# TFMV/quiver

Measured on AMD Instinct MI355X. Metric: flat_cosine_qps_recall_1.0, higher is better.
Workload: dtype f64; 1 GPU; flat cosine scan 10000000x768 fp32, k=10, single query per step, recall 1.0 (exact, bit-identical to the CPU oracle); rows_total=10000000, rows_per_gpu=10000000, dim=768, k=10, scan_streams=1, device=AMD Radeon Graphics (gfx950:sramecc+:xnack-), cus=256, rccl_ranks_seen=0

## Files before the change

### quiver_amd/csrc/qv_bound_scan.hip

```cpp
#include "qv_kernels.h"
#include "qv_bound.h"

namespace qv {

typedef uint32_t u4 __attribute__((ext_vector_type(4)));
constexpr uint32_t kBoundCandCap = 4096;
constexpr uint32_t kBoundMaxDim = 4096;
struct BoundCtrl { uint32_t thr_inv, cand_cnt, ticket, flag; };

template <int U, bool QN>
__device__ __forceinline__ void bound_block(const u4* __restrict__ p, const float* __restrict__ q_lds, uint32_t s0, float& acc, double& qa) {
    u4 x[2 * U];
#pragma unroll
    for (int u = 0; u < U; u++) {
        x[2 * u] = __builtin_nontemporal_load(&p[(size_t)(s0 + u) * 128]);
        x[2 * u + 1] = __builtin_nontemporal_load(&p[(size_t)(s0 + u) * 128 + 32]);
    }
    __builtin_amdgcn_sched_barrier(0);
#pragma unroll
    for (int u = 0; u < U; u++) {
        const f4* qq = reinterpret_cast<const f4*>(q_lds + (size_t)(s0 + u) * 16);
#pragma unroll
        for (int h = 0; h < 2; h++) {
            const u4 w = x[2 * u + h];
            const f4 qa4 = qq[2 * h], qb4 = qq[2 * h + 1];
            const float qe[8] = {qa4.x, qa4.y, qa4.z, qa4.w, qb4.x, qb4.y, qb4.z, qb4.w};
            const uint32_t ww[4] = {w.x, w.y, w.z, w.w};
#pragma unroll
            for (int j = 0; j < 4; j++) {
                acc = __builtin_fmaf(qe[2 * j], __uint_as_float(ww[j] << 16), acc);
                acc = __builtin_fmaf(qe[2 * j + 1], __uint_as_float(ww[j] & 0xFFFF0000u), acc);
                if constexpr (QN) { const double a = (double)qe[2 * j], b = (double)qe[2 * j + 1]; qa = __builtin_fma(a, a, qa); qa = __builtin_fma(b, b, qa); }
            }
        }
    }
}
template <bool QN>
__device__ __forceinline__ float bound_tile(const u4* __restrict__ p, const float* __restrict__ q_lds, uint32_t steps, double* qn2) {
    float acc = 0.f; double qa = 0.0;
    uint32_t s = 0;
    for (; s + 8 <= steps; s += 8) bound_block<8, QN>(p, q_lds, s, acc, qa);
    if (s + 4 <= steps) { bound_block<4, QN>(p, q_lds, s, acc, qa); s += 4; }
    if (s + 2 <= steps) { bound_block<2, QN>(p, q_lds, s, acc, qa); s += 2; }
    if (s < steps) bound_block<1, QN>(p, q_lds, s, acc, qa);
    if constexpr (QN) *qn2 = qa;
    return acc;
}

__device__ __forceinline__ bool bound_scan_tail(uint64_t list, uint64_t thr, uint64_t* wl , uint32_t wave, uint32_t lane, uint32_t k, BoundCtrl* __restrict__ ctrl,
                                                uint64_t* __restrict__ partial, uint32_t* __restrict__ seed_rows, float* __restrict__ seed_dist) {
    __shared__ uint32_t s_last;
    const uint32_t kth = k - 1;
    wl[wave * 64 + lane] = list;
    __syncthreads();
    if (wave == 0) {
        for (uint32_t w = 1; w < kScanWaves; w++) list_insert(list, thr, lane < k ? wl[w * 64 + lane] : kDeadKey, kth, lane);
        uint64_t* mine = partial + (size_t)blockIdx.x * k;
        if (lane < k) (void)atomicExch(reinterpret_cast<unsigned long long*>(&mine[lane]), (unsigned long long)list);
        asm volatile("s_waitcnt vmcnt(0)" ::: "memory");
        uint32_t last = 0;
        if (lane == 0) last = atomicAdd(&ctrl->ticket, 1u) == gridDim.x - 1 ? 1u : 0u;
        last = __builtin_amdgcn_readfirstlane(last);
        if (last && lane == 0) ctrl->ticket = 0;
        if (lane == 0) s_last = last;
    }
    __syncthreads();
    if (!s_last) return false;
    merge_lists_last_workgroup(partial, gridDim.x, k, seed_rows, seed_dist);
    if (wave == 0 && lane == kth) {
        const uint32_t o = ord_f32(seed_dist[kth]);
        ctrl->thr_inv = (seed_rows[kth] != 0xFFFFFFFFu && o < 0xFF800000u) ? ~o : 0u;
        ctrl->cand_cnt = 0;
    }
    return true;
}

template <int M, bool SKIP = false>
__global__ void __launch_bounds__(kScanBlock)
k_bound_scan(IndexView v, const float* __restrict__ query, uint32_t k, BoundCtrl* __restrict__ ctrl, uint32_t* __restrict__ lo_all ,
             uint64_t* __restrict__ partial , uint32_t* __restrict__ seed_rows, float* __restrict__ seed_dist,
             const uint32_t* __restrict__ gate = nullptr ) {
    if (gate != nullptr && *gate == 0u) return;
    extern __shared__ __align__(16) unsigned char smem[];
    float* q_lds = reinterpret_cast<float*>(smem);
    uint64_t* wl = reinterpret_cast<uint64_t*>(smem + (size_t)v.dim * sizeof(float));
    const uint32_t lane = lane_id();
    const uint32_t wave = __builtin_amdgcn_readfirstlane(threadIdx.x >> 6);
    for (uint32_t i = threadIdx.x; i < v.dim; i += blockDim.x) q_lds[i] = query[i];
    __syncthreads();
    const uint32_t steps = v.dim >> 4, tw = gridDim.x * kScanWaves, kth = k - 1;
    const double gamma = bound_scan_gamma(v.dim);
    const u4* plane = reinterpret_cast<const u4*>(v.plane) + ((lane >> 5) * 64 + (lane & 31));
    uint64_t list = kDeadKey, thr = kDeadKey;
    double qn = 0.0;

    uint64_t am_read = 0ull;
    auto finish_tile = [&](uint32_t t, float s, bool first) {
        const uint32_t row = t * 64 + lane;
        const double rn = v.rnorm[row];
        const float rr = v.rres[row];
        uint64_t am;
        if constexpr (SKIP) am = am_read; else am = v.alive[t];
        float lo, hi;
        (void)bound_scan_interval<M>(s, qn, rn, rr, v.dim, gamma, lo, hi);
        const bool live = (am >> lane) & 1ull;
        __builtin_nontemporal_store(live ? ord_f32(lo) : 0xFFFFFFFFu, &lo_all[row]);
        const uint64_t key = live ? (((uint64_t)ord_f32(hi) << 32) | row) : kDeadKey;
        if (first) { list = wave_sort64(key, lane); thr = readlane64(list, kth); }
        else list_insert(list, thr, key, kth, lane);
    };

    uint32_t t = blockIdx.x * kScanWaves + wave;
    if constexpr (SKIP) {
        bool first = true;
        uint64_t am_next = t < v.n_tiles ? v.alive[t] : 0ull;
        for (; t < v.n_tiles; t += tw) {
            const uint64_t am = am_next;
            if (t + tw < v.n_tiles) am_next = v.alive[t + tw];
            if (am == 0ull) { __builtin_nontemporal_store(0xFFFFFFFFu, &lo_all[t * 64 + lane]); continue; }
            am_read = am;
            if (first) {
                double qn2 = 0.0;
                const float s = bound_tile<true>(plane + (size_t)t * steps * 128, q_lds, steps, &qn2);
                qn = __builtin_sqrt(qn2);
                finish_tile(t, s, true);
                first = false;
            } else finish_tile(t, bound_tile<false>(plane + (size_t)t * steps * 128, q_lds, steps, nullptr), false);
        }
    } else {
        if (t < v.n_tiles) {
            double qn2 = 0.0;
            const float s = bound_tile<true>(plane + (size_t)t * steps * 128, q_lds, steps, &qn2);
            qn = __builtin_sqrt(qn2);
            finish_tile(t, s, true);
            t += tw;
        }
        for (; t < v.n_tiles; t += tw) finish_tile(t, bound_tile<false>(plane + (size_t)t * steps * 128, q_lds, steps, nullptr), false);
    }

    (void)bound_scan_tail(list, thr, wl, wave, lane, k, ctrl, partial, seed_rows, seed_dist);
}

__device__ __forceinline__ void bound_collect(const uint32_t* __restrict__ lo, uint32_t n , uint32_t H, uint32_t* __restrict__ cnt, uint32_t* __restrict__ cand,
                                              uint32_t cap = kBoundCandCap, const uint32_t* __restrict__ ids = nullptr) {
    const uint32_t lane = lane_id();
    for (uint32_t base = blockIdx.x * 1024u; base < n; base += gridDim.x * 1024u) {
        const uint32_t i = base + threadIdx.x * 4u;
        u4 x = {0xFFFFFFFFu, 0xFFFFFFFFu, 0xFFFFFFFFu, 0xFFFFFFFFu};
        if (i < n) x = __builtin_nontemporal_load(reinterpret_cast<const u4*>(lo + i));
        const uint32_t xs[4] = {x.x, x.y, x.z, x.w};
#pragma unroll
        for (int j = 0; j < 4; j++) {
            const bool c = xs[j] <= H && xs[j] != 0xFFFFFFFFu;
            const uint64_t m = __ballot(c);
            if (m) {
                uint32_t b0 = 0;
                if (lane == (uint32_t)__builtin_ctzll(m)) b0 = atomicAdd(cnt, (uint32_t)__builtin_popcountll(m));
                b0 = __builtin_amdgcn_readlane(b0, (uint32_t)__builtin_ctzll(m));
                const uint32_t slot = b0 + (uint32_t)__builtin_popcountll(m & ((1ull << lane) - 1ull));
                if (c && slot < cap) cand[slot] = ids ? ids[i + (uint32_t)j] : i + (uint32_t)j;
            }
        }
    }
}
__global__ void __launch_bounds__(256)
k_bound_collect(const uint32_t* __restrict__ lo_all, uint32_t n , BoundCtrl* __restrict__ ctrl, uint32_t* __restrict__ cand,
                const uint32_t* __restrict__ gate = nullptr , uint32_t cap = kBoundCandCap,
                const uint32_t* __restrict__ n_ptr = nullptr ,
                const uint32_t* __restrict__ ids = nullptr ) {
    if (gate != nullptr && *gate == 0u) return;
    const uint32_t inv = ctrl->thr_inv;
    if (inv == 0u) return;
    if (n_ptr != nullptr) n = *n_ptr;
    bound_collect(lo_all, n, ~inv, &ctrl->cand_cnt, cand, cap, ids);
}

template <int M, typename F>
__device__ __forceinline__ void bound_rescore_query(const IndexView& v, const float* __restrict__ query, uint32_t k, uint32_t cnt, bool has_H, const uint32_t* __restrict__ cand,
                                                    uint32_t* __restrict__ rows_out, float* __restrict__ dist_out, F decided) {
    using Q = typename MT<M>::Q;
    extern __shared__ __align__(16) unsigned char smem[];
    Q* q_lds = reinterpret_cast<Q*>(smem);
    uint64_t* wl = reinterpret_cast<uint64_t*>(smem + (((size_t)v.dim4 * 4 * sizeof(Q)) + 15) / 16 * 16);
    __shared__ double s_qn;
    const uint32_t lane = lane_id();
    const uint32_t wave = __builtin_amdgcn_readfirstlane(threadIdx.x >> 6);
    const uint32_t ns = cnt < kBoundCandCap ? cnt : kBoundCandCap, kth = k - 1;
    stage_query<M>(q_lds, query, v.dim, v.dim4);
    __syncthreads();
    const f4* tiles = reinterpret_cast<const f4*>(v.tiles);
    if (wave == kScanWaves - 1) {
        double ma = 0.0;
        for (uint32_t i = 0; i < v.dim; i++) { const double a = (double)q_lds[i]; ma = __builtin_fma(a, a, ma); }
        if (lane == 0) s_qn = __builtin_sqrt(ma);
    }
    __syncthreads();
    const double qn = s_qn;
    const bool hand_back = cnt > kBoundCandCap || !has_H || !bound_scan_norm_ok(qn, v.dim);
    if (threadIdx.x == 0) decided(hand_back);
    if (hand_back) return;
    QConst qc; qc.qn = 0.0; qc.qn32 = 0.0f;
    if constexpr (M == QV_COSINE) qc.qn = qn;
    uint64_t list = kDeadKey, thr = kDeadKey;
    for (uint32_t base = wave * 64; base < ns; base += kScanWaves * 64) {
        const uint32_t i = base + lane;
        uint64_t key = kDeadKey;
        if (i < ns) {
            const uint32_t row = cand[i];
            const typename MT<M>::A acc = row_accumulate<M, kUnroll, false, true>(tiles + (size_t)(row >> 6) * v.dim4 * 64 + (row & 63), 64, q_lds, v.dim4);
            double rn = 0.0;
            if constexpr (MT<M>::needs_rnorm) rn = v.rnorm[row];
            key = make_key(finalize<M>(acc, qc, rn), row);
        }
        if (base == wave * 64) { list = wave_sort64(key, lane); thr = readlane64(list, kth); }
        else list_insert(list, thr, key, kth, lane);
    }
    __syncthreads();
    wl[wave * 64 + lane] = list;
    __syncthreads();
    if (wave == 0) {
        for (uint32_t w = 1; w < kScanWaves; w++) list_insert(list, thr, lane < k ? wl[w * 64 + lane] : kDeadKey, kth, lane);
        if (lane < k) {
            const bool dead = list == kDeadKey;
            rows_out[lane] = dead ? 0xFFFFFFFFu : (uint32_t)list;
            dist_out[lane] = dead ? __uint_as_float(0x7F800000u) : unord_f32((uint32_t)(list >> 32));
        }
    }
}

constexpr uint32_t kBoundRescoreGrid = 64;
constexpr uint32_t kBoundRefineGrid = 256;
template <int M, bool P8 = false>
__global__ void __launch_bounds__(kScanBlock)
k_bound_rescore(IndexView v, const float* __restrict__ query, uint32_t k, BoundCtrl* __restrict__ ctrl, const uint32_t* __restrict__ cand,
                uint32_t* __restrict__ stats, uint32_t* __restrict__ rows_out, float* __restrict__ dist_out, uint32_t* gate, BoundCtrl* next,
                uint64_t* __restrict__ partial ) {
    if (gate != nullptr && *gate == 0u) return;
    using Q = typename MT<M>::Q;
    extern __shared__ __align__(16) unsigned char smem[];
    Q* q_lds = reinterpret_cast<Q*>(smem);
    const size_t q_bytes = (((size_t)v.dim4 * 4 * sizeof(Q)) + 15) / 16 * 16;
    uint64_t* wl = reinterpret_cast<uint64_t*>(smem + q_bytes);
    float* rbuf = reinterpret_cast<float*>(smem + q_bytes + (size_t)kScanWaves * 64 * sizeof(uint64_t));
    __shared__ double s_qn;
    __shared__ uint32_t s_last;
    const uint32_t cnt = ctrl->cand_cnt, thr_inv = ctrl->thr_inv;
    const uint32_t lane = lane_id();
    const uint32_t wave = __builtin_amdgcn_readfirstlane(threadIdx.x >> 6);
    const uint32_t ns = cnt < kBoundCandCap ? cnt : kBoundCandCap, kth = k - 1;
    const uint32_t active = std::max(1u, std::min((uint32_t)gridDim.x, (ns + kScanWaves - 1) / kScanWaves));
    const bool idle = blockIdx.x >= active;
    if (idle) {
        if (threadIdx.x == 0) s_last = atomicAdd(&ctrl->ticket, 1u) == gridDim.x - 1 ? 1u : 0u;
        __syncthreads();
        if (!s_last) return;
    }
    stage_query<M>(q_lds, query, v.dim, v.dim4);
    __syncthreads();
    if (wave == kScanWaves - 1) {
        double ma = 0.0;
        for (uint32_t i = 0; i < v.dim; i++) { const double a = (double)q_lds[i]; ma = __builtin_fma(a, a, ma); }
        if (lane == 0) s_qn = __builtin_sqrt(ma);
    }
    __syncthreads();
    const double qn = s_qn;
    const bool hand_back = cnt > kBoundCandCap || thr_inv == 0u || !bound_scan_norm_ok(qn, v.dim);
    uint64_t list = kDeadKey, thr = kDeadKey;
    if (!hand_back && !idle) {
        QConst qc; qc.qn = 0.0; qc.qn32 = 0.0f;
        if constexpr (M == QV_COSINE) qc.qn = qn;
        const f4* tiles = reinterpret_cast<const f4*>(v.tiles);
        f4* mine = reinterpret_cast<f4*>(rbuf + (size_t)wave * v.dim4 * 4);
        bool first = true;
        for (uint32_t i = blockIdx.x * kScanWaves + wave; i < ns; i += active * kScanWaves) {
            const uint32_t row = cand[i];
            const f4* src = tiles + (size_t)(row >> 6) * v.dim4 * 64 + (row & 63);
            double rn = 0.0;
            if constexpr (MT<M>::needs_rnorm) rn = v.rnorm[row];
            for (uint32_t c0 = 0; c0 < v.dim4; c0 += 256) {
                f4 x[4];
#pragma unroll
                for (uint32_t u = 0; u < 4; u++) { const uint32_t c = c0 + u * 64 + lane; if (c < v.dim4) x[u] = __builtin_nontemporal_load(&src[(size_t)c * 64]); }
#pragma unroll
                for (uint32_t u = 0; u < 4; u++) { const uint32_t c = c0 + u * 64 + lane; if (c < v.dim4) mine[c] = x[u]; }
            }
            __builtin_amdgcn_fence(__ATOMIC_RELEASE, "wavefront");
            __builtin_amdgcn_wave_barrier();
            __builtin_amdgcn_fence(__ATOMIC_ACQUIRE, "wavefront");
            typename MT<M>::A acc = 0;
            for (uint32_t c = 0; c < v.dim4; c++) {
                const f4 r = mine[c];
                const Q* qq = q_lds + (size_t)c * 4;
                acc1<M>(acc, qq[0], r.x); acc1<M>(acc, qq[1], r.y); acc1<M>(acc, qq[2], r.z); acc1<M>(acc, qq[3], r.w);
            }
            __builtin_amdgcn_fence(__ATOMIC_RELEASE, "wavefront");
            __builtin_amdgcn_wave_barrier();
            const uint64_t key = lane == 0 ? make_key(finalize<M>(acc, qc, rn), row) : kDeadKey;
            if (first) { list = wave_sort64(key, lane); thr = readlane64(list, kth); first = false; }
            else list_insert(list, thr, key, kth, lane);
        }
    }
    wl[wave * 64 + lane] = list;
    __syncthreads();
    if (wave == 0 && !idle) {
        if (!hand_back) {
            for (uint32_t w = 1; w < kScanWaves; w++) list_insert(list, thr, lane < k ? wl[w * 64 + lane] : kDeadKey, kth, lane);
            uint64_t* out = partial + (size_t)blockIdx.x * k;
            if (lane < k) (void)atomicExch(reinterpret_cast<unsigned long long*>(&out[lane]), (unsigned long long)list);
            asm volatile("s_waitcnt vmcnt(0)" ::: "memory");
        }
        uint32_t last = 0;
        if (lane == 0) last = atomicAdd(&ctrl->ticket, 1u) == gridDim.x - 1 ? 1u : 0u;
        last = __builtin_amdgcn_readfirstlane(last);
        if (lane == 0) s_last = last;
    }
    __syncthreads();
    if (!s_last) return;
    if (threadIdx.x == 0) {
        ctrl->ticket = 0;
        if constexpr (P8) {
            stats[kBound8StatsWord] = cnt;
            if (hand_back) (void)atomicAdd(&stats[kBound8StatsWord + 1], 1u);
            (void)atomicAdd(&stats[kBound8StatsWord + 2], 1u);
            if (!hand_back) { stats[0] = cnt; (void)atomicAdd(&stats[2], 1u); next->flag = 0u; }
        } else {
            stats[0] = cnt;
            if (hand_back) (void)atomicAdd(&stats[1], 1u);
            (void)atomicAdd(&stats[2], 1u);
            if (gate != nullptr) *gate = 0u;
        }
        ctrl->flag = hand_back ? 1u : 0u;
        ctrl->cand_cnt = 0; ctrl->thr_inv = 0;
    }
    if (hand_back) return;
    merge_lists_last_workgroup(partial, active, k, rows_out, dist_out);
}

typedef int i32;
template <int U>
__device__ __forceinline__ void bound8_block(const u4* __restrict__ p, const u4* __restrict__ qh, const u4* __restrict__ ql, uint32_t s0, i32 (&acc)[4]) {
    u4 x[U];
#pragma unroll
// ... 45 lines not shown
    double r2 = 0.0;
    int qs = 0;
    for (uint32_t i = threadIdx.x; i < dim; i += blockDim.x) {
        const double x = q_ok ? (double)query[i] : 0.0;
        const double qq = __builtin_rint(x / sq);
        const double hi = __builtin_rint(qq * (1.0 / 128.0)), lo = qq - 128.0 * hi;
        qh8[i] = (int8_t)(int)hi; ql8[i] = (int8_t)(int)lo;
        if constexpr (SUM) qs += (int)qq;
        const double d = x - sq * qq;
        r2 = __builtin_fma(d, d, r2);
    }
    r2 = wave_sum_f64(r2);
    if (lane == 0) s_res[wave] = r2;
    if constexpr (SUM) {
#pragma unroll
        for (int m = 32; m >= 1; m >>= 1) qs += __shfl_xor(qs, m);
        if (lane == 0) s_sum[wave] = qs;
    }
    if (wave == kScanWaves - 1) {
        double ma = 0.0;
        for (uint32_t b = 0; b < dim; b += 64) {
            const float x = b + lane < dim ? query[b + lane] : 0.f;
            const uint32_t n = dim - b < 64u ? dim - b : 64u;
            for (uint32_t j = 0; j < n; j++) { const double a = (double)__uint_as_float(__builtin_amdgcn_readlane(__float_as_uint(x), j)); ma = __builtin_fma(a, a, ma); }
        }
        if (lane == 0) s_qn = __builtin_sqrt(ma);
    }
    __syncthreads();
    double qres2 = 0.0;
    for (uint32_t w = 0; w < kScanWaves; w++) qres2 += s_res[w];
    qn_out = s_qn;
    sq_out = sq;
    qres_out = q_ok ? __builtin_sqrt(qres2) * (1.0 + 1e-9) + 1e-300 : __builtin_nan("");
    qsum_out = 0;
    if constexpr (SUM) { for (uint32_t w = 0; w < kScanWaves; w++) qsum_out += (long long)s_sum[w]; }
}

template <int M, bool SKIP = false>
__global__ void __launch_bounds__(kScanBlock)
k_bound_scan8(IndexView v, const float* __restrict__ query, uint32_t k, BoundCtrl* __restrict__ ctrl, uint32_t* __restrict__ lo_all ,
              uint64_t* __restrict__ partial , uint32_t* __restrict__ seed_rows, float* __restrict__ seed_dist) {
    extern __shared__ __align__(16) unsigned char smem[];
    int8_t* qh8 = reinterpret_cast<int8_t*>(smem);
    int8_t* ql8 = qh8 + v.dim;
    uint64_t* wl = reinterpret_cast<uint64_t*>(smem + (size_t)v.dim * 2);
    const uint32_t lane = lane_id();
    const uint32_t wave = __builtin_amdgcn_readfirstlane(threadIdx.x >> 6);
    const uint32_t steps = v.dim >> 4, tw = gridDim.x * kScanWaves;
    double sq, qn, qres; long long qsum;
    bound8_stage_query<false>(query, v.dim, qh8, ql8, lane, wave, sq, qn, qres, qsum);

    const u4* qh = reinterpret_cast<const u4*>(qh8);
    const u4* ql = reinterpret_cast<const u4*>(ql8);
    const u4* plane = reinterpret_cast<const u4*>(v.plane8) + lane;
    const uint32_t kth = k - 1;
    uint64_t list = kDeadKey, thr = kDeadKey;
    bool first = true;
    uint32_t t = blockIdx.x * kScanWaves + wave;
    uint64_t am_next = 0ull;
    if constexpr (SKIP) am_next = t < v.n_tiles ? v.alive[t] : 0ull;
    for (; t < v.n_tiles; t += tw) {
        uint64_t am;
        if constexpr (SKIP) {
            am = am_next;
            if (t + tw < v.n_tiles) am_next = v.alive[t + tw];
            if (am == 0ull) { __builtin_nontemporal_store(0xFFFFFFFFu, &lo_all[t * 64 + lane]); continue; }
        }
        const uint32_t row = t * 64 + lane;
        const double rn = v.rnorm[row];
        const float sc = v.rscale8[row], rr = v.rres8[row];
        if constexpr (!SKIP) am = v.alive[t];
        const long long isum = bound8_tile(plane + (size_t)t * steps * 64, qh, ql, steps);
        float lo, hi;
        (void)bound_scan_interval8<M>(isum, sq, qn, qres, rn, sc, rr, v.dim, lo, hi);
        const bool live = (am >> lane) & 1ull;
        __builtin_nontemporal_store(live ? ord_f32(lo) : 0xFFFFFFFFu, &lo_all[row]);
        const uint64_t key = live ? (((uint64_t)ord_f32(hi) << 32) | row) : kDeadKey;
        if (first) { list = wave_sort64(key, lane); thr = readlane64(list, kth); first = false; }
        else list_insert(list, thr, key, kth, lane);
    }
    (void)bound_scan_tail(list, thr, wl, wave, lane, k, ctrl, partial, seed_rows, seed_dist);
}

struct BoundQuery8 { double sq, qn, qres, pad; int8_t terms[2 * kBoundMaxDim]; };
template <int U>
__device__ __forceinline__ void bound6_block(const u4* __restrict__ p, const u4* __restrict__ qh, const u4* __restrict__ ql, uint32_t g0, i32 (&acc)[4]) {
    u4 x[3 * U];
#pragma unroll
    for (int u = 0; u < 3 * U; u++) x[u] = __builtin_nontemporal_load(&p[((size_t)g0 * 3 + u) * 64]);
    __builtin_amdgcn_sched_barrier(0);
#pragma unroll
    for (int u = 0; u < U; u++) {
        const uint32_t X[4] = {x[3 * u].x, x[3 * u].y, x[3 * u].z, x[3 * u].w};
        const uint32_t Y[4] = {x[3 * u + 1].x, x[3 * u + 1].y, x[3 * u + 1].z, x[3 * u + 1].w};
        const uint32_t Z[4] = {x[3 * u + 2].x, x[3 * u + 2].y, x[3 * u + 2].z, x[3 * u + 2].w};
        uint32_t c[4][4];
#pragma unroll
        for (int j = 0; j < 4; j++) {
            c[0][j] = X[j] & 0x3F3F3F3Fu; c[1][j] = Y[j] & 0x3F3F3F3Fu; c[2][j] = Z[j] & 0x3F3F3F3Fu;
            c[3][j] = ((X[j] >> 6) & 0x03030303u) | ((Y[j] >> 4) & 0x0C0C0C0Cu) | ((Z[j] >> 2) & 0x30303030u);
        }
#pragma unroll
        for (int st = 0; st < 4; st++) {
            const u4 h = qh[(g0 + u) * 4 + st], l = ql[(g0 + u) * 4 + st];
            acc[0] = __builtin_amdgcn_sdot4((i32)h.x, (i32)c[st][0], acc[0], false);
            acc[1] = __builtin_amdgcn_sdot4((i32)h.y, (i32)c[st][1], acc[1], false);
            acc[0] = __builtin_amdgcn_sdot4((i32)h.z, (i32)c[st][2], acc[0], false);
            acc[1] = __builtin_amdgcn_sdot4((i32)h.w, (i32)c[st][3], acc[1], false);
            acc[2] = __builtin_amdgcn_sdot4((i32)l.x, (i32)c[st][0], acc[2], false);
            acc[3] = __builtin_amdgcn_sdot4((i32)l.y, (i32)c[st][1], acc[3], false);
            acc[2] = __builtin_amdgcn_sdot4((i32)l.z, (i32)c[st][2], acc[2], false);
            acc[3] = __builtin_amdgcn_sdot4((i32)l.w, (i32)c[st][3], acc[3], false);
        }
    }
}
__device__ __forceinline__ long long bound6_tile(const u4* __restrict__ p, const u4* __restrict__ qh, const u4* __restrict__ ql, uint32_t groups) {
    i32 acc[4] = {0, 0, 0, 0};
    uint32_t g = 0;
    for (; g + 6 <= groups; g += 6) bound6_block<6>(p, qh, ql, g, acc);
    if (g + 3 <= groups) { bound6_block<3>(p, qh, ql, g, acc); g += 3; }
    if (g + 2 <= groups) { bound6_block<2>(p, qh, ql, g, acc); g += 2; }
    if (g < groups) bound6_block<1>(p, qh, ql, g, acc);
    return ((long long)acc[0] + (long long)acc[1]) * 128ll + ((long long)acc[2] + (long long)acc[3]);
}

template <int M>
__global__ void __launch_bounds__(kScanBlock)
k_bound_scan6(IndexView v, const float* __restrict__ query, uint32_t k, BoundCtrl* __restrict__ ctrl, uint32_t* __restrict__ lo_all ,
              uint64_t* __restrict__ partial , uint32_t* __restrict__ seed_rows, float* __restrict__ seed_dist,
              BoundQuery8* __restrict__ qst ) {
    extern __shared__ __align__(16) unsigned char smem[];
    int8_t* qh8 = reinterpret_cast<int8_t*>(smem);
    int8_t* ql8 = qh8 + v.dim;
    uint64_t* wl = reinterpret_cast<uint64_t*>(smem + (size_t)v.dim * 2);
    const uint32_t lane = lane_id();
    const uint32_t wave = __builtin_amdgcn_readfirstlane(threadIdx.x >> 6);
    const uint32_t groups = v.dim >> 6, tw = gridDim.x * kScanWaves;
    double sq, qn, qres; long long qsum;
    bound8_stage_query<true>(query, v.dim, qh8, ql8, lane, wave, sq, qn, qres, qsum);
    const long long bias = (long long)kBound6Bias * qsum;
    if (blockIdx.x == 0) {
        for (uint32_t i = threadIdx.x; i < v.dim / 8; i += blockDim.x) reinterpret_cast<u4*>(qst->terms)[i] = reinterpret_cast<const u4*>(smem)[i];
        if (threadIdx.x == 0) { qst->sq = sq; qst->qn = qn; qst->qres = qres; }
    }

    const u4* qh = reinterpret_cast<const u4*>(qh8);
    const u4* ql = reinterpret_cast<const u4*>(ql8);
    const u4* plane = reinterpret_cast<const u4*>(v.plane6) + lane;
    const uint32_t kth = k - 1;
    uint64_t list = kDeadKey, thr = kDeadKey;
    bool first = true;
    for (uint32_t t = blockIdx.x * kScanWaves + wave; t < v.n_tiles; t += tw) {
        const uint32_t row = t * 64 + lane;
        const double rn = v.rnorm[row];
        const float sc = 4.0f * v.rscale8[row], rr = v.rres6[row];
        const uint64_t am = v.alive[t];
        const long long isum = bound6_tile(plane + (size_t)t * groups * 192, qh, ql, groups) - bias;
        float lo, hi;
        (void)bound_scan_interval8<M>(isum, sq, qn, qres, rn, sc, rr, v.dim, lo, hi);
        const bool live = (am >> lane) & 1ull;
        __builtin_nontemporal_store(live ? ord_f32(lo) : 0xFFFFFFFFu, &lo_all[row]);
        const uint64_t key = live ? (((uint64_t)ord_f32(hi) << 32) | row) : kDeadKey;
        if (first) { list = wave_sort64(key, lane); thr = readlane64(list, kth); first = false; }
        else list_insert(list, thr, key, kth, lane);
    }
    (void)bound_scan_tail(list, thr, wl, wave, lane, k, ctrl, partial, seed_rows, seed_dist);
}
// ... 487 lines not shown
    for (int c = 0; c < 3; c++) {
        const BoundFloor &b = kBoundFloor[kRulesBf16][c], &l = kBoundFloor[kRulesBf16L2][c], &p = kBoundFloor[kRulesPlane8][c];
        const BoundFilterFloor& pf = kBoundFilterFloor[kRulesPlane8][c];
        if (p.wide_rows < b.wide_rows || p.wide_rows < l.wide_rows || p.narrow_dim < b.narrow_dim || p.narrow_dim < l.narrow_dim) return false;
        if (p.narrow_rows != 0 && (p.narrow_rows < b.narrow_rows || p.narrow_rows < l.narrow_rows)) return false;
        if (pf.min_dim < kBound8MinDim || (pf.min_rows != 0 && pf.min_rows < p.wide_rows)) return false;
    }
    return true;
}
static_assert(bound_floors_nest(), "the 8-bit floors are never below the bound scan's own, class by class, and its filtered floors never below its unfiltered ones");
static int rule_metric(const IndexView& v) { return v.metric == QV_L2 && v.l2_planes ? QV_RULE_L2_PLANES : v.metric; }
BoundAsk bound_ask(const IndexView& v, uint32_t nq, uint32_t k, uint32_t candidate_tiles) {
    return {rule_metric(v), v.dim, v.n_rows, nq, k, candidate_tiles, v.plane != nullptr, v.plane8 != nullptr, v.plane8 != nullptr && v.plane6 != nullptr};
}
BoundKnobs bound_knobs(const IndexView& v) { return {v.bound_scan, {v.bound_plane, v.bound_plane_filtered, v.bound_plane_mq, v.bound_plane_filtered_mq}, v.bound_plane6}; }
int bound_scan_mode(int mode) { static const int env_mode = env_int("QV_BOUND_SCAN", 0); return mode ? mode : env_mode; }
static int bound_plane_mode(BoundForm form, int mode) {
    static const int env_mode[4] = {env_int("QV_BOUND_PLANE", 0), env_int("QV_BOUND_PLANE_FILTERED", 0), env_int("QV_BOUND_PLANE_MQ", 0), env_int("QV_BOUND_PLANE_FILTERED_MQ", 0)};
    return mode ? mode : env_mode[form];
}
bool bound_scan_kernels_serve(const BoundAsk& a) {
    const uint32_t n_tiles = (a.n_rows + 63) / 64;
    const bool metric_ok = a.rule_metric == QV_COSINE || a.rule_metric == QV_DOT || a.rule_metric == QV_RULE_L2_PLANES;
    if (a.nq < 1 || a.nq > kBoundMqMax || a.k < 1 || a.k > (uint32_t)kMaxFusedK || !metric_ok || !a.has_plane) return false;
    if ((a.dim & 15u) != 0 || a.dim > kBoundMaxDim || n_tiles < 8) return false;
    return a.nq == 1 || (uint64_t)a.nq * n_tiles * 256 <= (2ull << 30);
}
static bool bound_auto(const BoundAsk& a, int rules) {
    const int cls = a.nq == 1 ? 0 : a.nq <= 4 ? 1 : 2;
    const BoundFloor& f = kBoundFloor[rules][cls];
    const uint32_t floor = a.dim >= kBoundWideDim ? f.wide_rows : a.dim >= f.narrow_dim ? f.narrow_rows : 0u;
    if (floor == 0 || a.n_rows < floor) return false;
    if (a.candidate_tiles == kBoundNoFilter) return true;
    const BoundFilterFloor& g = kBoundFilterFloor[rules][cls];
    const uint64_t n_tiles = ((uint64_t)a.n_rows + 63) / 64, ct = std::min<uint64_t>(a.candidate_tiles, n_tiles);
    if (ct == 0 || a.dim < g.min_dim || g.min_rows == 0 || a.n_rows < g.min_rows) return false;
    const bool big = g.big_rows != 0 && a.n_rows >= g.big_rows;
    return ct * 10 >= n_tiles * (big ? g.big_tenths : g.tenths) && (big || g.small_k == 0 || a.k <= g.small_k);
}
static bool bound6_auto(const BoundAsk& a) {
    if (!bound_auto(a, kRulesPlane8)) return false;
    const uint32_t floor = a.dim >= kBound6MaxDim ? 0u : a.dim >= kBoundWideDim ? kBound6MinRows : a.dim >= kBound6NarrowDim ? kBound6NarrowRows : 0u;
    return floor != 0 && a.n_rows >= floor && a.k <= kBound6MaxK;
}
BoundStages bound_scan_decide(const BoundAsk& a, const BoundKnobs& knobs) {
    const int scan = bound_scan_mode(knobs.scan);
    if (scan == 2 || !bound_scan_kernels_serve(a)) return BoundStages::none;
    if (scan != 1 && !bound_auto(a, a.rule_metric == QV_RULE_L2_PLANES ? kRulesBf16L2 : kRulesBf16)) return BoundStages::none;
    const int plane = bound_plane_mode(bound_form(a), knobs.plane[bound_form(a)]);
    if (plane == 2 || !a.has_plane8) return BoundStages::bf16;
    if (plane != 1 && !bound_auto(a, kRulesPlane8)) return BoundStages::bf16;
    if (bound_form(a) != bound_one || !a.has_plane6 || (a.dim & 63u) != 0) return BoundStages::plane8_first;
    static const int env6 = env_int("QV_BOUND_PLANE6", 0);
    const int plane6 = knobs.plane6 ? knobs.plane6 : env6;
    if (plane6 == 2) return BoundStages::plane8_first;
    return plane6 == 1 || bound6_auto(a) ? BoundStages::plane6_first : BoundStages::plane8_first;
}
struct BoundLayout { uint64_t* partial; uint32_t* seed_rows; float* seed_dist; uint32_t *cand, *cand6, *n8; BoundQuery8* qst; uint32_t* lo_all; size_t end, total; };
static BoundLayout bound_layout(void* base, const ScanPlan& p, uint32_t k, uint32_t n_tiles, WsLog* log = nullptr) {
    WsCarver w{static_cast<char*>(base), 0, 0, log};
    BoundLayout L{};
    L.partial = w.take256<uint64_t>((size_t)p.grid * k);
    L.seed_rows = w.take<uint32_t>(64);
    L.seed_dist = w.take<float>(64);
    L.cand = w.take<uint32_t>(kBoundCandCap);
    L.cand6 = w.take<uint32_t>(kBound6CandCap);
    L.n8 = w.take<uint32_t>(64);
    L.qst = w.take<BoundQuery8>(1);
    L.lo_all = w.take<uint32_t>((size_t)n_tiles * 64);
    return w.finish(L);
}
size_t bound_scan_workspace_bytes(const ScanPlan& p, uint32_t k, uint32_t n_tiles, WsLog* log) { return bound_layout(nullptr, p, k, n_tiles, log).total; }
hipError_t launch_bound_scan(const IndexView& v, const ScanPlan& p, const float* d_query, uint32_t k, void* d_ws, uint32_t* d_ctrl, uint32_t* d_stats,
                             uint32_t* d_rows_out, float* d_dist_out, const uint32_t** gate_out, hipStream_t s, bool masked, bool plane8_first, bool plane6_first) {
    if (!bound_scan_kernels_serve(bound_ask(v, 1, k, kBoundNoFilter)) || !d_ctrl || !d_stats) return hipErrorInvalidValue;
    if (plane8_first && !v.plane8) return hipErrorInvalidValue;
    if (plane6_first && (!plane8_first || masked || !v.plane6 || !v.rres6 || (v.dim & 63u) != 0)) return hipErrorInvalidValue;
    const uint32_t grid = p.grid;
    const BoundLayout L = bound_layout(d_ws, p, k, v.n_tiles);
    uint64_t* partial = L.partial;
    uint32_t *seed_rows = L.seed_rows, *cand = L.cand, *cand6 = L.cand6, *n8 = L.n8, *lo_all = L.lo_all;
    float* seed_dist = L.seed_dist;
    BoundQuery8* qst = L.qst;
    const uint32_t n_pad = v.n_tiles * 64, cgrid = std::min(1024u, (n_pad + 1023u) / 1024u);
    BoundCtrl* ctrl = reinterpret_cast<BoundCtrl*>(d_ctrl);
    const size_t lds1 = (size_t)v.dim * sizeof(float) + (size_t)kScanWaves * 64 * sizeof(uint64_t);
    const size_t lds2 = query_lds_bytes(v.metric, v.dim4) + (size_t)kScanWaves * 64 * sizeof(uint64_t) + (size_t)kScanWaves * v.dim4 * 4 * sizeof(float);
    const uint32_t rgrid = std::min(kBoundRescoreGrid, grid);
    const size_t lds8 = (size_t)v.dim * 2 + (size_t)kScanWaves * 64 * sizeof(uint64_t);
    auto run = [&](auto Mc, auto Mk) -> hipError_t {
        constexpr int M = decltype(Mc)::value;
        constexpr bool MASKED = decltype(Mk)::value;
        const uint32_t* const no_gate = nullptr;
        auto attrs = [&](auto scan, size_t lds_scan, auto rescore) -> hipError_t {
            const hipError_t e = set_lds(scan, lds_scan);
            return e != hipSuccess ? e : set_lds(rescore, lds2);
        };
        auto stage = [&](auto scan, size_t lds_scan, auto rescore, BoundCtrl* c, uint32_t* gate, BoundCtrl* next, auto... scan_gate) {
            hipLaunchKernelGGL(scan, dim3(grid), dim3(kScanBlock), lds_scan, s, v, d_query, k, c, lo_all, partial, seed_rows, seed_dist, scan_gate...);
            hipLaunchKernelGGL(k_bound_collect, dim3(cgrid), dim3(256), 0, s, lo_all, n_pad, c, cand, (const uint32_t*)gate, kBoundCandCap, no_gate, no_gate);
            hipLaunchKernelGGL(rescore, dim3(rgrid), dim3(kScanBlock), lds2, s, v, d_query, k, c, cand, d_stats, d_rows_out, d_dist_out, gate, next, partial);
        };
        hipError_t e = attrs(k_bound_scan<M, MASKED>, lds1, k_bound_rescore<M>);
        if (e == hipSuccess && plane8_first) e = attrs(k_bound_scan8<M, MASKED>, lds8, k_bound_rescore<M, true>);
        if constexpr (!MASKED) {
            if (e == hipSuccess && plane6_first) e = set_lds(k_bound_scan6<M>, lds8);
            if (e == hipSuccess && plane6_first) e = set_lds(k_bound_refine8<M>, lds8);
        }
        if (e != hipSuccess) return e;
        if (plane6_first) {
            if constexpr (!MASKED) {
                BoundCtrl *ctrl8 = ctrl + 1, *ctrl6 = ctrl + 2;
                uint32_t* gate8 = &ctrl8->flag;
                const uint32_t fgrid = std::min(kBoundRefineGrid, grid), cgrid8 = std::min(cgrid, kBound6CandCap / 1024u);
                hipLaunchKernelGGL(k_bound_scan6<M>, dim3(grid), dim3(kScanBlock), lds8, s, v, d_query, k, ctrl6, lo_all, partial, seed_rows, seed_dist, qst);
                hipLaunchKernelGGL(k_bound_collect, dim3(cgrid), dim3(256), 0, s, lo_all, n_pad, ctrl6, cand6, no_gate, kBound6CandCap, no_gate, no_gate);
                hipLaunchKernelGGL(k_bound_refine8<M>, dim3(fgrid), dim3(kScanBlock), lds8, s, v, (const BoundQuery8*)qst, k, ctrl6, ctrl8, cand6, lo_all, n8, partial, seed_rows, seed_dist, d_stats);
                hipLaunchKernelGGL(k_bound_collect, dim3(cgrid8), dim3(256), 0, s, lo_all, 0u, ctrl8, cand, no_gate, kBoundCandCap, (const uint32_t*)n8, (const uint32_t*)cand6);
                hipLaunchKernelGGL((k_bound_rescore<M, true>), dim3(rgrid), dim3(kScanBlock), lds2, s, v, d_query, k, ctrl8, cand, d_stats, d_rows_out, d_dist_out, (uint32_t*)nullptr, ctrl, partial);
                stage(k_bound_scan<M, MASKED>, lds1, k_bound_rescore<M>, ctrl, gate8, (BoundCtrl*)nullptr, (const uint32_t*)gate8);
            }
        } else if (plane8_first) {
            BoundCtrl* ctrl8 = ctrl + 1;
            uint32_t* gate8 = &ctrl8->flag;
            stage(k_bound_scan8<M, MASKED>, lds8, k_bound_rescore<M, true>, ctrl8, (uint32_t*)nullptr, ctrl);
            stage(k_bound_scan<M, MASKED>, lds1, k_bound_rescore<M>, ctrl, gate8, (BoundCtrl*)nullptr, (const uint32_t*)gate8);
        } else stage(k_bound_scan<M, MASKED>, lds1, k_bound_rescore<M>, ctrl, (uint32_t*)nullptr, (BoundCtrl*)nullptr, no_gate);
        return hipSuccess;
    };
    auto run_metric = [&](auto Mk) -> hipError_t {
        return v.metric == QV_COSINE ? run(std::integral_constant<int, QV_COSINE>{}, Mk)
             : v.metric == QV_DOT  ? run(std::integral_constant<int, QV_DOT>{}, Mk) : run(std::integral_constant<int, QV_L2>{}, Mk);
    };
    const hipError_t e = masked ? run_metric(std::true_type{}) : run_metric(std::false_type{});
    if (e != hipSuccess) return e;
    *gate_out = &ctrl->flag;
    return hipGetLastError();
}
int host_bound_interval(int metric, uint32_t dim, float s, double qn, double rn, float rres, float* d_lo, float* d_hi) {
    const double gamma = bound_scan_gamma(dim);
    const bool sure = metric == QV_COSINE ? bound_scan_interval<QV_COSINE>(s, qn, rn, rres, dim, gamma, *d_lo, *d_hi)
                    : metric == QV_DOT  ? bound_scan_interval<QV_DOT>(s, qn, rn, rres, dim, gamma, *d_lo, *d_hi)
                                        : bound_scan_interval<QV_L2>(s, qn, rn, rres, dim, gamma, *d_lo, *d_hi);
    return sure ? 0 : 1;
}

int host_bound_interval8(int metric, uint32_t dim, long long isum, double sq, double qn, double qres, double rn, float rscale, float rres8, float* d_lo, float* d_hi) {
    const bool sure = metric == QV_COSINE ? bound_scan_interval8<QV_COSINE>(isum, sq, qn, qres, rn, rscale, rres8, dim, *d_lo, *d_hi)
                    : metric == QV_DOT  ? bound_scan_interval8<QV_DOT>(isum, sq, qn, qres, rn, rscale, rres8, dim, *d_lo, *d_hi)
                                        : bound_scan_interval8<QV_L2>(isum, sq, qn, qres, rn, rscale, rres8, dim, *d_lo, *d_hi);
    return sure ? 0 : 1;
}
int host_quantize_row8(uint32_t dim, const float* row, int8_t* out_bytes, float* out_scale, float* out_res) {
    float maxabs = 0.f; bool bad = false; double n2 = 0.0;
    for (uint32_t i = 0; i < dim; i++) {
        bad |= !((row[i] - row[i]) == 0.0f);
        maxabs = __builtin_fmaxf(maxabs, __builtin_fabsf(row[i]));
        n2 = __builtin_fma((double)row[i], (double)row[i], n2);
    }
    const float scale = bad ? 0.0f : bound8_scale(maxabs);
    double s2 = 0.0;
    for (uint32_t i = 0; i < dim; i++) {
        const int b = scale > 0.0f ? bound8_quant(row[i], scale) : 0;
        const double d = (double)row[i] - (double)scale * (double)b;
        s2 = __builtin_fma(d, d, s2);
        out_bytes[i] = (int8_t)b;
    }
    *out_scale = scale;
    *out_res = bound8_row_res(bad, maxabs, n2, s2, dim);
    return 0;
}

int host_quantize_row6(uint32_t dim, const float* row, float scale8, uint8_t* out_bytes, float* out_res) {
    float maxabs = 0.f; bool bad = false; double n2 = 0.0;
    for (uint32_t i = 0; i < dim; i++) {
        bad |= !((row[i] - row[i]) == 0.0f);
        maxabs = __builtin_fmaxf(maxabs, __builtin_fabsf(row[i]));
        n2 = __builtin_fma((double)row[i], (double)row[i], n2);
    }
    const float div = scale8 > 0.0f ? scale8 : 1.0f;
    const double step = 4.0 * (double)scale8;
    double s2 = 0.0;
    for (uint32_t g = 0; g < dim / 64; g++) {
        uint8_t piece[48] = {};
        for (uint32_t d = 0; d < 64; d++) {
            const float x = row[g * 64 + d];
            const int q = scale8 > 0.0f ? bound6_quant(x, div) : 0;
            const double e = (double)x - step * (double)q;
            s2 = __builtin_fma(e, e, s2);
            bound6_pack(piece, d, (uint32_t)(q + kBound6Bias));
        }
        for (uint32_t i = 0; i < 48; i++) out_bytes[g * 48 + i] = piece[i];
    }
    const float res8 = bound8_row_res(bad, maxabs, n2, 0.0, dim);
    *out_res = res8 == res8 ? bound8_res_up(s2) : __builtin_nanf("");
    return 0;
}
int host_unpack_row6(uint32_t dim, const uint8_t* bytes, uint8_t* out_codes) {
    for (uint32_t g = 0; g < dim / 64; g++) {
        uint8_t piece[48];
        for (uint32_t i = 0; i < 48; i++) piece[i] = bytes[g * 48 + i];
        for (uint32_t d = 0; d < 64; d++) out_codes[g * 64 + d] = (uint8_t)bound6_unpack(piece, d);
    }
    return 0;
}

struct BoundMqLayout { uint64_t* partial; uint32_t* seed_rows; float* seed_dist; uint32_t* flags; double* qnorm; float* qblk; uint32_t *cand, *lo_all; void* redo_ws; size_t end, total; };
static BoundMqLayout bound_mq_layout(void* base, const ScanPlan& p, uint32_t nq, uint32_t k, uint32_t n_tiles, uint32_t dim, WsLog* log = nullptr) {
    WsCarver w{static_cast<char*>(base), 0, 0, log};
    BoundMqLayout L{};
    L.partial = w.take256<uint64_t>((size_t)nq * p.grid * k);
    L.seed_rows = w.take256<uint32_t>((size_t)kBoundMqMax * 64);
    L.seed_dist = w.take256<float>((size_t)kBoundMqMax * 64);
    L.flags = w.take<uint32_t>(64);
    L.qnorm = w.take<double>(32);
    L.qblk = w.take256<float>((size_t)dim * kBoundMqMax);
    WsCarver redo = w.overlay();
    L.cand = w.take<uint32_t>((size_t)nq * kBoundCandCap);
    L.lo_all = w.take<uint32_t>((size_t)nq * n_tiles * 64);
    L.redo_ws = redo.take<char>(redo_workspace_bytes(p, nq, k));
    w.cover(redo);
    return w.finish(L);
}
size_t bound_scan_mq_workspace_bytes(const ScanPlan& p, uint32_t nq, uint32_t k, uint32_t n_tiles, uint32_t dim, WsLog* log) { return bound_mq_layout(nullptr, p, nq, k, n_tiles, dim, log).total; }
hipError_t launch_bound_scan_mq(const IndexView& v, const ScanPlan& p, const float* d_queries, uint32_t nq, uint32_t k, void* d_ws, uint32_t* d_ctrl, uint32_t* d_stats,
                                uint32_t* d_rows_out, float* d_dist_out, hipStream_t s, const RowSetRef* h_sets, bool plane8_first) {
    if (nq < 2 || !bound_scan_kernels_serve(bound_ask(v, nq, k, kBoundNoFilter)) || !d_ctrl || !d_stats) return hipErrorInvalidValue;
    if (plane8_first && !v.plane8) return hipErrorInvalidValue;
    BoundSetTable tab;
    for (uint32_t i = 0; i < kBoundSets; i++) tab.e[i] = h_sets && i < nq ? h_sets[i] : RowSetRef{nullptr, 0, 0};
    if (h_sets && trace_filtered()) {
        if (plane8_first) fprintf(stderr, "qv: scan kernel = k_bound_scan8_mq sets QB=%d, then gated k_bound_scan_mq sets (nq=%u, tiles=%u)\n", nq <= 4 ? 4 : 8, nq, v.n_tiles);
        else fprintf(stderr, "qv: scan kernel = k_bound_scan_mq sets QB=%d (nq=%u, tiles=%u)\n", nq <= 4 ? 4 : 8, nq, v.n_tiles);
    }
    const uint32_t grid = p.grid;
    const BoundMqLayout L = bound_mq_layout(d_ws, p, nq, k, v.n_tiles, v.dim);
    uint64_t* partial = L.partial;
    uint32_t *seed_rows = L.seed_rows, *flags = L.flags, *cand = L.cand, *lo_all = L.lo_all;
    float *seed_dist = L.seed_dist, *qblk = L.qblk;
    double* qnorm = L.qnorm;
    void* redo_ws = L.redo_ws;
    const uint32_t n_pad = v.n_tiles * 64, cgrid = std::min(1024u, (n_pad + 1023u) / 1024u);
    BoundCtrl* ctrl = reinterpret_cast<BoundCtrl*>(d_ctrl);
    const size_t lds2 = query_lds_bytes(v.metric, v.dim4) + (size_t)kScanWaves * 64 * sizeof(uint64_t);
    hipError_t e = hipSuccess;
    static_assert(2 * kBoundMaxDim * kBoundMqMax <= kBoundMaxDim * kBoundMqMax * sizeof(float) && 3 * kBoundMqMax * sizeof(double) <= 256 &&
                  (kBound8MqHandWord + kBoundMqMax + 1) * 4 <= 256, "the 8-bit stage's terms, scalars and hand-on words fit the bfloat16 stage's");
    uint32_t* hand = flags + kBound8MqHandWord;
    const uint32_t* gate = plane8_first ? hand + kBoundMqMax : nullptr;
    const uint32_t* hand_in = plane8_first ? hand : nullptr;
    auto run = [&](auto Mc, auto Qc, auto Sc) -> hipError_t {
        constexpr int M = decltype(Mc)::value, QB = decltype(Qc)::value;
        constexpr bool SETS = decltype(Sc)::value;
        SetsArg<SETS> sets{};
        if constexpr (SETS) sets = tab;
        const size_t lds1 = (size_t)kScanWaves * QB * 64 * sizeof(uint64_t);
        e = set_lds(k_bound_rescore_mq<M>, lds2);
        if (e == hipSuccess && plane8_first) e = set_lds((k_bound_rescore_mq<M, 1>), lds2);
        if (e == hipSuccess && plane8_first) e = set_lds((k_bound_rescore_mq<M, 2>), lds2);
        if (e != hipSuccess) return e;
        if (plane8_first) {
            hipLaunchKernelGGL((k_bound_prep8_mq<QB>), dim3(QB), dim3(kScanBlock), 0, s, d_queries, nq, v.dim, reinterpret_cast<int8_t*>(qblk), qnorm, hand, d_stats);
            hipLaunchKernelGGL((k_bound_scan8_mq<M, QB, SETS>), dim3(grid), dim3(kScanBlock), lds1, s, v, reinterpret_cast<const u4*>(qblk), qnorm, nq, k, lo_all, partial, sets);
            e = launch_merge_lists(partial, grid, nq, k, seed_rows, seed_dist, s);
            if (e != hipSuccess) return e;
            hipLaunchKernelGGL(k_bound_collect_mq, dim3(cgrid, nq), dim3(256), 0, s, lo_all, n_pad, k, seed_rows, seed_dist, ctrl, cand, (const uint32_t*)nullptr);
            hipLaunchKernelGGL((k_bound_rescore_mq<M, 1>), dim3(nq), dim3(kScanBlock), lds2, s, v, d_queries, k, seed_rows, seed_dist, ctrl, cand, flags, d_stats, d_rows_out, d_dist_out, hand);
        }
        hipLaunchKernelGGL((k_bound_prep_mq<QB>), dim3((v.dim * QB + 255) / 256 + QB), dim3(256), 0, s, d_queries, nq, v.dim, qblk, qnorm, d_stats, gate);
        hipLaunchKernelGGL((k_bound_scan_mq<M, QB, SETS>), dim3(grid), dim3(kScanBlock), lds1, s, v, qblk, qnorm, nq, k, lo_all, partial, sets, gate);
        e = launch_merge_lists(partial, grid, nq, k, seed_rows, seed_dist, s, gate);
        if (e != hipSuccess) return e;
        hipLaunchKernelGGL(k_bound_collect_mq, dim3(cgrid, nq), dim3(256), 0, s, lo_all, n_pad, k, seed_rows, seed_dist, ctrl, cand, hand_in);
        if (plane8_first) hipLaunchKernelGGL((k_bound_rescore_mq<M, 2>), dim3(nq), dim3(kScanBlock), lds2, s, v, d_queries, k, seed_rows, seed_dist, ctrl, cand, flags, d_stats, d_rows_out, d_dist_out, hand);
        else hipLaunchKernelGGL((k_bound_rescore_mq<M>), dim3(nq), dim3(kScanBlock), lds2, s, v, d_queries, k, seed_rows, seed_dist, ctrl, cand, flags, d_stats, d_rows_out, d_dist_out, (uint32_t*)nullptr);
        return hipSuccess;
    };
    auto run_sets = [&](auto Mc, auto Qc) -> hipError_t { return h_sets ? run(Mc, Qc, std::true_type{}) : run(Mc, Qc, std::false_type{}); };
    auto run_qb = [&](auto Mc) -> hipError_t { return nq <= 4 ? run_sets(Mc, std::integral_constant<int, 4>{}) : run_sets(Mc, std::integral_constant<int, 8>{}); };
    e = v.metric == QV_COSINE ? run_qb(std::integral_constant<int, QV_COSINE>{})
      : v.metric == QV_DOT  ? run_qb(std::integral_constant<int, QV_DOT>{}) : run_qb(std::integral_constant<int, QV_L2>{});
    if (e != hipSuccess) return e;
    e = hipGetLastError();
    if (e != hipSuccess) return e;
    return launch_flat_redo_flagged(v, p, d_queries, nq, k, k, flags, redo_ws, d_rows_out, d_dist_out, s, h_sets);
}

}
```

Before: 900.6 queries/s.

## Buffer collect candidates in LDS with prefetch and reuse precomputed query norm

Rewrites the candidate-collect kernel so each block processes two vectors per thread per chunk with software prefetch of the next chunk. Survivors go into a shared-memory buffer and are flushed with one global atomic per flush, where before each wave ballot issued its own global atomic. The collect grid is capped at 512 blocks. The rescore kernel can also take the query norm from the 8-bit stage's precomputed query state instead of recomputing it serially. The aim is less global atomic contention, better latency hiding over the 10M-entry bound array, and one less serial dot product, at the cost of extra block barriers and more complex control flow.

```diff
diff --git a/quiver_amd/csrc/qv_bound_scan.hip b/quiver_amd/csrc/qv_bound_scan.hip
--- a/quiver_amd/csrc/qv_bound_scan.hip
+++ b/quiver_amd/csrc/qv_bound_scan.hip
@@ -7,6 +7,7 @@
 constexpr uint32_t kBoundCandCap = 4096;
 constexpr uint32_t kBoundMaxDim = 4096;
 struct BoundCtrl { uint32_t thr_inv, cand_cnt, ticket, flag; };
+struct BoundQuery8 { double sq, qn, qres, pad; int8_t terms[2 * kBoundMaxDim]; };
 
 template <int U, bool QN>
 __device__ __forceinline__ void bound_block(const u4* __restrict__ p, const float* __restrict__ q_lds, uint32_t s0, float& acc, double& qa) {
@@ -141,27 +142,82 @@
     (void)bound_scan_tail(list, thr, wl, wave, lane, k, ctrl, partial, seed_rows, seed_dist);
 }
 
+constexpr uint32_t kCollectVecs = 2;
+constexpr uint32_t kCollectChunk = kCollectVecs * 1024;
+constexpr uint32_t kCollectBuf = kCollectChunk + kCollectChunk / 2;
+#ifndef QV_COLLECT_GRID
+#define QV_COLLECT_GRID 512u
+#endif
+constexpr uint32_t kBoundCollectGrid = QV_COLLECT_GRID;
 __device__ __forceinline__ void bound_collect(const uint32_t* __restrict__ lo, uint32_t n , uint32_t H, uint32_t* __restrict__ cnt, uint32_t* __restrict__ cand,
                                               uint32_t cap = kBoundCandCap, const uint32_t* __restrict__ ids = nullptr) {
+    __shared__ uint32_t s_rows[kCollectBuf];
+    __shared__ uint32_t s_cnt[3], s_base;
     const uint32_t lane = lane_id();
-    for (uint32_t base = blockIdx.x * 1024u; base < n; base += gridDim.x * 1024u) {
-        const uint32_t i = base + threadIdx.x * 4u;
-        u4 x = {0xFFFFFFFFu, 0xFFFFFFFFu, 0xFFFFFFFFu, 0xFFFFFFFFu};
-        if (i < n) x = __builtin_nontemporal_load(reinterpret_cast<const u4*>(lo + i));
-        const uint32_t xs[4] = {x.x, x.y, x.z, x.w};
-#pragma unroll
-        for (int j = 0; j < 4; j++) {
-            const bool c = xs[j] <= H && xs[j] != 0xFFFFFFFFu;
-            const uint64_t m = __ballot(c);
-            if (m) {
-                uint32_t b0 = 0;
-                if (lane == (uint32_t)__builtin_ctzll(m)) b0 = atomicAdd(cnt, (uint32_t)__builtin_popcountll(m));
-                b0 = __builtin_amdgcn_readlane(b0, (uint32_t)__builtin_ctzll(m));
-                const uint32_t slot = b0 + (uint32_t)__builtin_popcountll(m & ((1ull << lane) - 1ull));
-                if (c && slot < cap) cand[slot] = ids ? ids[i + (uint32_t)j] : i + (uint32_t)j;
-            }
-        }
-    }
+    const uint32_t stride = gridDim.x * kCollectChunk, mine = threadIdx.x * 4u;
+    if (threadIdx.x < 3u) s_cnt[threadIdx.x] = 0;
+    __syncthreads();
+    auto flush = [&](uint32_t fill, bool more) {
+        if (threadIdx.x == 0) s_base = atomicAdd(cnt, fill);
+        __syncthreads();
+        const uint32_t b0 = s_base;
+        for (uint32_t i = threadIdx.x; i < fill; i += blockDim.x) {
+            if (b0 + i < cap) cand[b0 + i] = ids ? ids[s_rows[i]] : s_rows[i];
+        }
+        if (more) __syncthreads();
+    };
+    const u4 none = {0xFFFFFFFFu, 0xFFFFFFFFu, 0xFFFFFFFFu, 0xFFFFFFFFu};
+    uint32_t base = blockIdx.x * kCollectChunk;
+    uint32_t fill = 0, p = 0;
+    bool x_on[kCollectVecs]; u4 x[kCollectVecs];
+#pragma unroll
+    for (uint32_t v = 0; v < kCollectVecs; v++) {
+        x_on[v] = base < n && n - base > v * 1024u + mine;
+        x[v] = __builtin_nontemporal_load(reinterpret_cast<const u4*>(lo + (x_on[v] ? base + v * 1024u + mine : 0u)));
+    }
+    while (base < n) {
+        const bool more = n - base > stride;
+        bool nx_on[kCollectVecs]; u4 nx[kCollectVecs];
+#pragma unroll
+        for (uint32_t v = 0; v < kCollectVecs; v++) {
+            nx_on[v] = more && n - base - stride > v * 1024u + mine;
+            nx[v] = __builtin_nontemporal_load(reinterpret_cast<const u4*>(lo + (nx_on[v] ? base + stride + v * 1024u + mine : 0u)));
+        }
+        __builtin_amdgcn_sched_barrier(0);
+        bool c[kCollectVecs * 4]; uint64_t m[kCollectVecs * 4];
+        uint32_t tot = 0;
+#pragma unroll
+        for (uint32_t v = 0; v < kCollectVecs; v++) {
+            if (!x_on[v]) x[v] = none;
+            const uint32_t xs[4] = {x[v].x, x[v].y, x[v].z, x[v].w};
+#pragma unroll
+            for (int j = 0; j < 4; j++) {
+                c[v * 4 + j] = xs[j] <= H && xs[j] != 0xFFFFFFFFu;
+                m[v * 4 + j] = __ballot(c[v * 4 + j]);
+                tot += (uint32_t)__builtin_popcountll(m[v * 4 + j]);
+            }
+        }
+        if (tot) {
+            uint32_t b0 = 0;
+            if (lane == 0) b0 = atomicAdd(&s_cnt[p], tot);
+            b0 = fill + __builtin_amdgcn_readfirstlane(b0);
+#pragma unroll
+            for (uint32_t e = 0; e < kCollectVecs * 4; e++) {
+                if (c[e]) s_rows[b0 + (uint32_t)__builtin_popcountll(m[e] & ((1ull << lane) - 1ull))] = base + (e >> 2) * 1024u + mine + (e & 3u);
+                b0 += (uint32_t)__builtin_popcountll(m[e]);
+            }
+        }
+        __syncthreads();
+        fill += s_cnt[p];
+        if (threadIdx.x == 0) s_cnt[p == 0u ? 2u : p - 1u] = 0;
+        p = p == 2u ? 0u : p + 1u;
+        if (!more) break;
+        if (fill > kCollectBuf - kCollectChunk) { flush(fill, true); fill = 0; }
+#pragma unroll
+        for (uint32_t v = 0; v < kCollectVecs; v++) { x[v] = nx[v]; x_on[v] = nx_on[v]; }
+        base += stride;
+    }
+    if (fill) flush(fill, false);
 }
 __global__ void __launch_bounds__(256)
 k_bound_collect(const uint32_t* __restrict__ lo_all, uint32_t n , BoundCtrl* __restrict__ ctrl, uint32_t* __restrict__ cand,
@@ -234,7 +290,8 @@
 __global__ void __launch_bounds__(kScanBlock)
 k_bound_rescore(IndexView v, const float* __restrict__ query, uint32_t k, BoundCtrl* __restrict__ ctrl, const uint32_t* __restrict__ cand,
                 uint32_t* __restrict__ stats, uint32_t* __restrict__ rows_out, float* __restrict__ dist_out, uint32_t* gate, BoundCtrl* next,
-                uint64_t* __restrict__ partial ) {
+                uint64_t* __restrict__ partial ,
+                const BoundQuery8* __restrict__ qst = nullptr ) {
     if (gate != nullptr && *gate == 0u) return;
     using Q = typename MT<M>::Q;
     extern __shared__ __align__(16) unsigned char smem[];
@@ -257,7 +314,9 @@
     }
     stage_query<M>(q_lds, query, v.dim, v.dim4);
     __syncthreads();
-    if (wave == kScanWaves - 1) {
+    if (qst != nullptr) {
+        if (threadIdx.x == 0) s_qn = qst->qn;
+    } else if (wave == kScanWaves - 1) {
         double ma = 0.0;
         for (uint32_t i = 0; i < v.dim; i++) { const double a = (double)q_lds[i]; ma = __builtin_fma(a, a, ma); }
         if (lane == 0) s_qn = __builtin_sqrt(ma);
@@ -469,7 +528,6 @@
     (void)bound_scan_tail(list, thr, wl, wave, lane, k, ctrl, partial, seed_rows, seed_dist);
 }
 
-struct BoundQuery8 { double sq, qn, qres, pad; int8_t terms[2 * kBoundMaxDim]; };
 template <int U>
 __device__ __forceinline__ void bound6_block(const u4* __restrict__ p, const u4* __restrict__ qh, const u4* __restrict__ ql, uint32_t g0, i32 (&acc)[4]) {
     u4 x[3 * U];
@@ -1123,7 +1181,7 @@
     uint32_t *seed_rows = L.seed_rows, *cand = L.cand, *cand6 = L.cand6, *n8 = L.n8, *lo_all = L.lo_all;
     float* seed_dist = L.seed_dist;
     BoundQuery8* qst = L.qst;
-    const uint32_t n_pad = v.n_tiles * 64, cgrid = std::min(1024u, (n_pad + 1023u) / 1024u);
+    const uint32_t n_pad = v.n_tiles * 64, cgrid = std::min(kBoundCollectGrid, (n_pad + kCollectChunk - 1u) / kCollectChunk);
     BoundCtrl* ctrl = reinterpret_cast<BoundCtrl*>(d_ctrl);
     const size_t lds1 = (size_t)v.dim * sizeof(float) + (size_t)kScanWaves * 64 * sizeof(uint64_t);
     const size_t lds2 = query_lds_bytes(v.metric, v.dim4) + (size_t)kScanWaves * 64 * sizeof(uint64_t) + (size_t)kScanWaves * v.dim4 * 4 * sizeof(float);
@@ -1140,7 +1198,7 @@
         auto stage = [&](auto scan, size_t lds_scan, auto rescore, BoundCtrl* c, uint32_t* gate, BoundCtrl* next, auto... scan_gate) {
             hipLaunchKernelGGL(scan, dim3(grid), dim3(kScanBlock), lds_scan, s, v, d_query, k, c, lo_all, partial, seed_rows, seed_dist, scan_gate...);
             hipLaunchKernelGGL(k_bound_collect, dim3(cgrid), dim3(256), 0, s, lo_all, n_pad, c, cand, (const uint32_t*)gate, kBoundCandCap, no_gate, no_gate);
-            hipLaunchKernelGGL(rescore, dim3(rgrid), dim3(kScanBlock), lds2, s, v, d_query, k, c, cand, d_stats, d_rows_out, d_dist_out, gate, next, partial);
+            hipLaunchKernelGGL(rescore, dim3(rgrid), dim3(kScanBlock), lds2, s, v, d_query, k, c, cand, d_stats, d_rows_out, d_dist_out, gate, next, partial, (const BoundQuery8*)nullptr);
         };
         hipError_t e = attrs(k_bound_scan<M, MASKED>, lds1, k_bound_rescore<M>);
         if (e == hipSuccess && plane8_first) e = attrs(k_bound_scan8<M, MASKED>, lds8, k_bound_rescore<M, true>);
@@ -1153,12 +1211,12 @@
             if constexpr (!MASKED) {
                 BoundCtrl *ctrl8 = ctrl + 1, *ctrl6 = ctrl + 2;
                 uint32_t* gate8 = &ctrl8->flag;
-                const uint32_t fgrid = std::min(kBoundRefineGrid, grid), cgrid8 = std::min(cgrid, kBound6CandCap / 1024u);
+                const uint32_t fgrid = std::min(kBoundRefineGrid, grid), cgrid8 = std::min(cgrid, kBound6CandCap / kCollectChunk);
                 hipLaunchKernelGGL(k_bound_scan6<M>, dim3(grid), dim3(kScanBlock), lds8, s, v, d_query, k, ctrl6, lo_all, partial, seed_rows, seed_dist, qst);
                 hipLaunchKernelGGL(k_bound_collect, dim3(cgrid), dim3(256), 0, s, lo_all, n_pad, ctrl6, cand6, no_gate, kBound6CandCap, no_gate, no_gate);
                 hipLaunchKernelGGL(k_bound_refine8<M>, dim3(fgrid), dim3(kScanBlock), lds8, s, v, (const BoundQuery8*)qst, k, ctrl6, ctrl8, cand6, lo_all, n8, partial, seed_rows, seed_dist, d_stats);
                 hipLaunchKernelGGL(k_bound_collect, dim3(cgrid8), dim3(256), 0, s, lo_all, 0u, ctrl8, cand, no_gate, kBoundCandCap, (const uint32_t*)n8, (const uint32_t*)cand6);
-                hipLaunchKernelGGL((k_bound_rescore<M, true>), dim3(rgrid), dim3(kScanBlock), lds2, s, v, d_query, k, ctrl8, cand, d_stats, d_rows_out, d_dist_out, (uint32_t*)nullptr, ctrl, partial);
+                hipLaunchKernelGGL((k_bound_rescore<M, true>), dim3(rgrid), dim3(kScanBlock), lds2, s, v, d_query, k, ctrl8, cand, d_stats, d_rows_out, d_dist_out, (uint32_t*)nullptr, ctrl, partial, (const BoundQuery8*)qst);
                 stage(k_bound_scan<M, MASKED>, lds1, k_bound_rescore<M>, ctrl, gate8, (BoundCtrl*)nullptr, (const uint32_t*)gate8);
             }
         } else if (plane8_first) {
@@ -1281,7 +1339,7 @@
     float *seed_dist = L.seed_dist, *qblk = L.qblk;
     double* qnorm = L.qnorm;
     void* redo_ws = L.redo_ws;
-    const uint32_t n_pad = v.n_tiles * 64, cgrid = std::min(1024u, (n_pad + 1023u) / 1024u);
+    const uint32_t n_pad = v.n_tiles * 64, cgrid = std::min(kBoundCollectGrid, (n_pad + kCollectChunk - 1u) / kCollectChunk);
     BoundCtrl* ctrl = reinterpret_cast<BoundCtrl*>(d_ctrl);
     const size_t lds2 = query_lds_bytes(v.metric, v.dim4) + (size_t)kScanWaves * 64 * sizeof(uint64_t);
     hipError_t e = hipSuccess;
```

After: 950.1 queries/s, median of 6. 5.5% higher.
